# a-to-the-5/Simple-MapReduce-Search-Engine-Information-Retrieval-

Hardware: AMD Instinct MI355X
Metric: index build GB/s of text (top-10 queries/sec in 'query') (higher is better)
Workload: dtype u8 text / int32 postings / f64 weights

## Files before the change

### simple-mapreduce-search-engine-information-retrieval-_amd/csrc/sme_sort.hip

```cpp
#include <hip/hip_runtime.h>

#include "sme_internal.hpp"

namespace sme {
namespace {

#ifndef SME_RSNT
#define SME_RSNT 512
#endif
constexpr int kRsNT = SME_RSNT;
constexpr int kRsWaves = kRsNT / 64;
constexpr int kRsIPL = 16;
constexpr int kRsTile = kRsNT * kRsIPL;
constexpr int kRsWaveItems = 64 * kRsIPL;
constexpr int kRsMaxBits = 11;
constexpr int kRsMaxBins = 1 << kRsMaxBits;
constexpr int kRsBPT = kRsMaxBins / kRsNT;
constexpr int kRsGroups = 1024;
constexpr int kRsScanSums = 1024;
constexpr int kRsOffTiles = 16;

struct RsGroups {
  int64_t tpg;
  int G;
};
static RsGroups rs_groups(int64_t ntiles) {
  const int64_t tpg = std::max<int64_t>(4, (ntiles + kRsGroups - 1) / kRsGroups);
  const int64_t g = (ntiles + tpg - 1) / tpg;
  return RsGroups{tpg, (int)((g + 15) / 16 * 16)};
}

struct Gather {
  const int64_t *reg, *xoff, *crec;
  int64_t nrec;
  const uint32_t *rval;
  int tf_shift;
};
__device__ __forceinline__ void gather_start(const Gather &g, int64_t x, int64_t &rec, int64_t &nx, int64_t &dl) {
  rec = g.crec[x >> 10];
  nx = g.xoff[rec + 1];
  dl = g.reg[rec] - g.xoff[rec];
}
__device__ __forceinline__ int64_t gather_pos(const Gather &g, int64_t x, int64_t &rec, int64_t &nx, int64_t &dl) {
  while (x >= nx) {
    rec++;
    nx = g.xoff[rec + 1];
    dl = g.reg[rec] - g.xoff[rec];
  }
  return x + dl;
}
constexpr int kGRec = 48;
__device__ __forceinline__ int64_t gather_table(const Gather &g, int64_t x0, int lane, int64_t *gx, int64_t *gdl,
                                                uint32_t *gv = nullptr) {
  const int64_t rec0 = g.crec[x0 >> 10];
  const int64_t r = rec0 + lane;
  if (lane < kGRec) {
    gx[lane] = r <= g.nrec ? g.xoff[r] : INT64_MAX;
    gdl[lane] = r < g.nrec ? g.reg[r] - g.xoff[r] : 0;
    if (gv) gv[lane] = r < g.nrec ? g.rval[r] : 0u;
  }
  if (lane == 0) gx[kGRec] = rec0 + kGRec <= g.nrec ? g.xoff[rec0 + kGRec] : INT64_MAX;
  __builtin_amdgcn_fence(__ATOMIC_SEQ_CST, "wavefront");
  __builtin_amdgcn_wave_barrier();
  return rec0;
}
__device__ __forceinline__ int64_t gather_at(const Gather &g, int64_t x, int &j, const int64_t *gx, const int64_t *gdl,
                                             int64_t rec0, uint32_t *jr = nullptr) {
#ifdef SME_RS_GATHER_CEIL
  if (jr) *jr = 0u;
  return x + gdl[0];
#endif
  while (j < kGRec - 1 && x >= gx[j + 1]) j++;
  if (x < gx[j + 1]) {
    if (jr) *jr = (uint32_t)j;
    return x + gdl[j];
  }
  int64_t rec = rec0 + kGRec - 1, nx = g.xoff[rec + 1], dl = g.reg[rec] - g.xoff[rec];
  const int64_t p = gather_pos(g, x, rec, nx, dl);
  if (jr) *jr = (uint32_t)(rec - rec0);
  return p;
}
__global__ void k_rs_chunk_rec(const int64_t *__restrict__ xoff, int64_t nrec, int64_t P, int64_t *__restrict__ crec) {
  for (int64_t c = blockIdx.x * (int64_t)blockDim.x + threadIdx.x; (c << 10) < P; c += (int64_t)gridDim.x * blockDim.x) {
    const int64_t x = c << 10;
    int64_t lo = 0, hi = nrec;
    while (hi - lo > 1) {
      const int64_t m = (lo + hi) >> 1;
      if (xoff[m] <= x) lo = m;
      else hi = m;
    }
    crec[c] = lo;
  }
}

__global__ __launch_bounds__(kRsNT) void k_rs_count(const uint32_t *__restrict__ key, int64_t P, int shift,
                                                    int nbins, uint32_t *__restrict__ counts, Gather g) {
  __shared__ uint32_t h[kRsMaxBins];
  const int tid = threadIdx.x;
  for (int b = tid; b < nbins; b += kRsNT) h[b] = 0;
  __syncthreads();
  const int64_t t0 = (int64_t)blockIdx.x * kRsTile;
  const uint32_t mask = (uint32_t)nbins - 1u;
  const int64_t n = min((int64_t)kRsTile, P - t0);
  if (g.reg != nullptr) {
    __shared__ int64_t gx_all[kRsWaves][kGRec + 1], gdl_all[kRsWaves][kGRec];
    const int lane = tid & 63, w = tid >> 6;
    const int64_t wb = t0 + (int64_t)w * kRsWaveItems;
    if (wb < P) {
      const int64_t rec0 = gather_table(g, wb, lane, gx_all[w], gdl_all[w]);
      int j = 0;
      uint32_t kk[kRsIPL];
#pragma unroll
      for (int s = 0; s < kRsIPL; s++) {
        const int64_t x = wb + s * 64 + lane;
        kk[s] = x < P ? key[gather_at(g, x, j, gx_all[w], gdl_all[w], rec0)] : 0u;
      }
#pragma unroll
      for (int s = 0; s < kRsIPL; s++)
        if (wb + s * 64 + lane < P) atomicAdd(&h[(kk[s] >> shift) & mask], 1u);
    }
  } else if (n == kRsTile) {
    const uint4 *k4 = reinterpret_cast<const uint4 *>(key + t0);
#pragma unroll
    for (int i = 0; i < kRsIPL / 4; i++) {
      const uint4 v = k4[i * kRsNT + tid];
      atomicAdd(&h[(v.x >> shift) & mask], 1u);
      atomicAdd(&h[(v.y >> shift) & mask], 1u);
      atomicAdd(&h[(v.z >> shift) & mask], 1u);
      atomicAdd(&h[(v.w >> shift) & mask], 1u);
    }
  } else {
    for (int64_t i = tid; i < n; i += kRsNT) atomicAdd(&h[(key[t0 + i] >> shift) & mask], 1u);
  }
  __syncthreads();
  for (int b = tid; b < nbins; b += kRsNT) counts[(int64_t)blockIdx.x * nbins + b] = h[b];
}

__global__ __launch_bounds__(kRsNT) void k_rs_colsum(const uint32_t *__restrict__ counts, int64_t ntiles, int nbins,
                                                     int64_t tpg, int G, uint32_t *__restrict__ gsum) {
  const int g = blockIdx.x;
  const int64_t ta = (int64_t)g * tpg, tb = min(ntiles, ta + tpg);
  for (int b = threadIdx.x; b < nbins; b += kRsNT) {
    uint32_t s = 0;
    for (int64_t t = ta; t < tb; t++) s += counts[t * nbins + b];
    gsum[(int64_t)b * G + g] = s;
  }
}

__global__ __launch_bounds__(kRsNT) void k_rs_scan(uint32_t *__restrict__ a, int n) {
  __shared__ uint32_t ws[kRsWaves];
  const int tid = threadIdx.x, lane = tid & 63, w = tid >> 6;
  uint32_t carry = 0;
  uint4 x[4];
  auto load = [&](int r0, uint4 *y) {
    const int i0 = r0 + 16 * tid;
#pragma unroll
    for (int c = 0; c < 4; c++) y[c] = i0 < n ? reinterpret_cast<const uint4 *>(a + i0)[c] : make_uint4(0, 0, 0, 0);
  };
  load(0, x);
  for (int r0 = 0; r0 < n; r0 += 16 * kRsNT) {
    const int i0 = r0 + 16 * tid;
    uint32_t s = 0;
#pragma unroll
    for (int c = 0; c < 4; c++) s += x[c].x + x[c].y + x[c].z + x[c].w;
    uint32_t incl = s;
    for (int o = 1; o < 64; o <<= 1) {
      const uint32_t u = __shfl_up(incl, o, 64);
      if (lane >= o) incl += u;
    }
    if (lane == 63) ws[w] = incl;
    uint4 xn[4];
    load(r0 + 16 * kRsNT, xn);
    __syncthreads();
    uint32_t wb = carry, tot = 0;
    for (int j = 0; j < kRsWaves; j++) {
      const uint32_t t = ws[j];
      if (j < w) wb += t;
      tot += t;
    }
    uint32_t run = wb + incl - s;
    if (i0 < n) {
#pragma unroll
      for (int c = 0; c < 4; c++) {
        uint4 y;
        y.x = run;
        run += x[c].x;
        y.y = run;
        run += x[c].y;
        y.z = run;
        run += x[c].z;
        y.w = run;
        run += x[c].w;
        reinterpret_cast<uint4 *>(a + i0)[c] = y;
      }
    }
    carry += tot;
    __syncthreads();
#pragma unroll
    for (int c = 0; c < 4; c++) x[c] = xn[c];
  }
}

__global__ __launch_bounds__(kRsNT) void k_rs_colscan(uint32_t *__restrict__ counts, int64_t ntiles, int nbins,
                                                      int64_t tpg, int G, const uint32_t *__restrict__ gsum) {
  const int g = blockIdx.x;
  const int64_t ta = (int64_t)g * tpg, tb = min(ntiles, ta + tpg);
  for (int b = threadIdx.x; b < nbins; b += kRsNT) {
    uint32_t run = gsum[(int64_t)b * G + g];
    for (int64_t t = ta; t < tb; t++) {
      const uint32_t c = counts[t * nbins + b];
      counts[t * nbins + b] = run;
      run += c;
    }
  }
}

template <bool LAST, bool PACK, bool KEYS = true>
__global__ __launch_bounds__(kRsNT) void k_rs_scatter(const uint32_t *__restrict__ key, const uint32_t *__restrict__ val,
                                                      int64_t P, int shift, int nbits,
                                                      const uint32_t *__restrict__ offs, uint32_t *__restrict__ okey,
                                                      uint32_t *__restrict__ oval, int32_t *__restrict__ odocno,
                                                      int32_t *__restrict__ otf, int64_t dmin, uint32_t F,
                                                      Gather g, const double *__restrict__ lut, double idf,
                                                      double *__restrict__ ow, const uint2 *__restrict__ xw) {
  __shared__ uint16_t wc[kRsWaves * kRsMaxBins];
  __shared__ uint32_t gd[kRsMaxBins];
  __shared__ uint32_t stage[kRsTile];
  __shared__ uint32_t ws[kRsWaves];
  const int tid = threadIdx.x, lane = tid & 63, w = tid >> 6;
  const int nbins = 1 << nbits;
  const uint32_t mask = (uint32_t)nbins - 1u;
  const int64_t per = (int64_t)(gridDim.x >> 3);
  const int64_t tile = (int64_t)(blockIdx.x & 7) * per + (blockIdx.x >> 3);
  const int64_t t0 = tile * kRsTile;
  if (t0 >= P) return;
  const int n = (int)min((int64_t)kRsTile, P - t0);
  for (int i = tid; i < kRsWaves * kRsMaxBins / 2; i += kRsNT) reinterpret_cast<uint32_t *>(wc)[i] = 0u;
  __syncthreads();
  uint16_t *mine = wc + w * kRsMaxBins;
  const int wb = w * kRsWaveItems;
  const uint64_t lt = (1ull << lane) - 1ull;
  uint32_t k[kRsIPL], v[kRsIPL], pos[kRsIPL];
  if (g.reg != nullptr) {
    __shared__ int64_t gx_all[kRsWaves][kGRec + 1], gdl_all[kRsWaves][kGRec];
    __shared__ uint32_t gv_all[kRsWaves][kGRec];
    uint32_t *gv = PACK ? gv_all[w] : nullptr;
    int64_t rec0 = 0;
    if (wb < n) rec0 = gather_table(g, t0 + wb, lane, gx_all[w], gdl_all[w], gv);
    int j = 0;
    if (PACK) {
      const uint32_t kmask = g.tf_shift >= 32 ? 0xFFFFFFFFu : (1u << g.tf_shift) - 1u;
#pragma unroll
      for (int s = 0; s < kRsIPL; s++) {
        const int i = wb + s * 64 + lane;
        k[s] = 0u;
        v[s] = 0u;
        if (i < n) k[s] = key[gather_at(g, t0 + i, j, gx_all[w], gdl_all[w], rec0, &v[s])];
      }
#pragma unroll
      for (int s = 0; s < kRsIPL; s++) {
        const uint32_t wd = k[s], jr = v[s];
        k[s] = wd & kmask;
        if (wb + s * 64 + lane < n)
          v[s] = (jr < (uint32_t)kGRec ? gv[jr] : g.rval[rec0 + jr]) + (uint32_t)((uint64_t)wd >> g.tf_shift);
      }
    } else {
#pragma unroll
      for (int s = 0; s < kRsIPL; s++) {
        const int i = wb + s * 64 + lane;
        k[s] = 0u;
        v[s] = 0u;
        if (i < n) {
          const int64_t p = gather_at(g, t0 + i, j, gx_all[w], gdl_all[w], rec0);
          k[s] = key[p];
          v[s] = val[p];
        }
      }
    }
  } else {
#pragma unroll
    for (int s = 0; s < kRsIPL; s++) {
      const int i = wb + s * 64 + lane;
      const bool ok = i < n;
      k[s] = ok ? key[t0 + i] : 0u;
      v[s] = ok ? val[t0 + i] : 0u;
    }
  }
#pragma unroll
  for (int s = 0; s < kRsIPL; s++) {
    const bool ok = wb + s * 64 + lane < n;
    const uint32_t d = (k[s] >> shift) & mask;
    uint64_t peers = (uint64_t)__ballot(ok);
    for (int b = 0; b < nbits; b++) {
      const bool bit = (d >> b) & 1u;
      const uint64_t m = (uint64_t)__ballot(bit);
      peers &= bit ? m : ~m;
    }
    uint32_t r = 0;
    if (ok) {
      const uint32_t c = mine[d];
      r = c + (uint32_t)__popcll(peers & lt);
      if ((peers & lt) == 0) mine[d] = (uint16_t)(c + (uint32_t)__popcll(peers));
    }
    pos[s] = r;
  }
  __syncthreads();
  {
    const int b0 = kRsBPT * tid;
    uint32_t tc[kRsBPT];
    uint32_t s2 = 0;
#pragma unroll
    for (int q = 0; q < kRsBPT; q++) {
      tc[q] = 0;
      if (b0 + q < nbins) {
#pragma unroll
        for (int x = 0; x < kRsWaves; x++) tc[q] += wc[x * kRsMaxBins + b0 + q];
      }
      s2 += tc[q];
    }
    uint32_t incl = s2;
    for (int o = 1; o < 64; o <<= 1) {
      const uint32_t u = __shfl_up(incl, o, 64);
      if (lane >= o) incl += u;
    }
    if (lane == 63) ws[w] = incl;
    __syncthreads();
    uint32_t ex = incl - s2;
    for (int j = 0; j < w; j++) ex += ws[j];
#pragma unroll
    for (int q = 0; q < kRsBPT; q++) {
      if (b0 + q < nbins) {
        uint32_t r = ex;
        gd[b0 + q] = offs[tile * nbins + b0 + q] - r;
#pragma unroll
        for (int x = 0; x < kRsWaves; x++) {
          const uint32_t c = wc[x * kRsMaxBins + b0 + q];
          wc[x * kRsMaxBins + b0 + q] = (uint16_t)r;
          r += c;
        }
      }
      ex += tc[q];
    }
  }
  __syncthreads();
#pragma unroll
  for (int s = 0; s < kRsIPL; s++) {
    if (wb + s * 64 + lane >= n) continue;
    pos[s] += mine[(k[s] >> shift) & mask];
    stage[pos[s]] = k[s];
  }
  __syncthreads();
  uint32_t dst[kRsIPL];
#pragma unroll
  for (int j = 0; j < kRsIPL; j++) {
    const int p = j * kRsNT + tid;
    if (p < n) {
      const uint32_t kk = stage[p];
      dst[j] = gd[(kk >> shift) & mask] + (uint32_t)p;
      if (LAST && xw) {
        const uint2 x = xw[kk];
        dst[j] += x.x;
        if (KEYS) okey[dst[j]] = x.y;
      } else if (KEYS) {
        okey[dst[j]] = kk;
      }
    }
  }
  __syncthreads();
#pragma unroll
  for (int s = 0; s < kRsIPL; s++)
    if (wb + s * 64 + lane < n) stage[pos[s]] = v[s];
  __syncthreads();
#pragma unroll
  for (int j = 0; j < kRsIPL; j++) {
    const int p = j * kRsNT + tid;
    if (p < n) {
      const uint32_t vv = stage[p];
      if (LAST) {
        odocno[dst[j]] = (int32_t)((int64_t)(vv / F) + dmin);
        otf[dst[j]] = (int32_t)(vv % F);
        if (ow) ow[dst[j]] = __dmul_rn(lut[vv % F], idf);
      } else {
        oval[dst[j]] = vv;
      }
    }
  }
}

__global__ __launch_bounds__(kRsNT) void k_rs_term_off(const uint32_t *__restrict__ key, int64_t P, int shift, int nbits,
                                                       const uint32_t *__restrict__ offs, int64_t V,
                                                       const uint2 *__restrict__ xw, int64_t *__restrict__ off,
                                                       int64_t vend, int64_t pend) {
  __shared__ uint32_t ks[kRsTile];
  __shared__ uint16_t sp[kRsTile];
  __shared__ uint32_t hist[kRsMaxBins];
  __shared__ uint32_t rc[kRsIPL * kRsWaves + 1];
  __shared__ uint32_t act;
  const int tid = threadIdx.x, lane = tid & 63, w = tid >> 6;
  const int nbins = 1 << nbits;
  const uint32_t mask = (uint32_t)nbins - 1u;
  const uint32_t lmask = (1u << shift) - 1u;
  if (blockIdx.x == 0 && tid == 0) off[vend] = pend;
  if (P <= 0) return;
  int64_t tile = 0;
  auto emit = [&](uint32_t L) {
    for (int d = tid; d < nbins; d += kRsNT) {
      const uint64_t k = ((uint64_t)d << shift) | L;
      if (k < (uint64_t)V) {
        const int64_t o = (int64_t)offs[tile * nbins + d] + hist[d];
        if (xw) {
          const uint2 x = xw[k];
          off[x.y] = o + x.x;
        } else {
          off[k] = o;
        }
      }
    }
  };
  if (shift == 0) {
    for (int b = tid; b < nbins; b += kRsNT) hist[b] = 0;
    __syncthreads();
    emit(0u);
    return;
  }
  if (tid == 0) act = 0u;
  __syncthreads();
  if (tid < kRsOffTiles) {
    const int64_t a0 = ((int64_t)blockIdx.x * kRsOffTiles + tid) * kRsTile;
    if (a0 < P) {
      const int64_t last = min(a0 + kRsTile, P) - 1;
      if (a0 == 0 || (key[a0 - 1] & lmask) != (key[last] & lmask)) atomicOr(&act, 1u << tid);
    }
  }
  __syncthreads();
  const uint64_t lt = (1ull << lane) - 1ull;
  for (uint32_t todo = act; todo != 0u; todo &= todo - 1u) {
    tile = (int64_t)blockIdx.x * kRsOffTiles + (__ffs(todo) - 1);
    const int64_t t0 = tile * kRsTile;
    const int n = (int)min((int64_t)kRsTile, P - t0);
    const uint32_t lprev = t0 > 0 ? key[t0 - 1] & lmask : 0u;
    for (int b = tid; b < nbins; b += kRsNT) hist[b] = 0;
    for (int p = tid; p < n; p += kRsNT) ks[p] = key[t0 + p];
    __syncthreads();
    uint32_t mine = 0;
#pragma unroll
    for (int j = 0; j < kRsIPL; j++) {
      const int p = j * kRsNT + tid;
      bool f = false;
      if (p < n) f = (ks[p] & lmask) != (p > 0 ? ks[p - 1] & lmask : lprev) || (p == 0 && t0 == 0);
      const uint64_t b = (uint64_t)__ballot(f);
      if (f) mine |= 1u << j;
      if (lane == 0) rc[j * kRsWaves + w] = (uint32_t)__popcll(b);
    }
    __syncthreads();
    if (w == 0) {
      const uint32_t a = rc[2 * lane], b = rc[2 * lane + 1];
      uint32_t incl = a + b;
      for (int o = 1; o < 64; o <<= 1) {
        const uint32_t u = __shfl_up(incl, o, 64);
        if (lane >= o) incl += u;
      }
      rc[2 * lane] = incl - a - b;
      rc[2 * lane + 1] = incl - b;
      if (lane == 63) rc[kRsIPL * kRsWaves] = incl;
    }
    __syncthreads();
#pragma unroll
    for (int j = 0; j < kRsIPL; j++) {
      const bool f = (mine >> j) & 1u;
      const uint64_t b = (uint64_t)__ballot(f);
      if (f) sp[rc[j * kRsWaves + w] + (uint32_t)__popcll(b & lt)] = (uint16_t)(j * kRsNT + tid);
    }
    __syncthreads();
    const int ns = (int)rc[kRsIPL * kRsWaves];
    int pos = 0;
    for (int si = 0; si < ns; si++) {
      const int s = sp[si];
      for (int p = pos + tid; p < s; p += kRsNT) atomicAdd(&hist[(ks[p] >> shift) & mask], 1u);
      __syncthreads();
      emit(ks[s] & lmask);
      __syncthreads();
      pos = s;
    }
    __syncthreads();
  }
}

template <typename K>
__global__ __launch_bounds__(kRsNT) void k_kv_count(const K *__restrict__ key, int64_t n, int shift, int nbins,
                                                    uint32_t *__restrict__ counts) {
  __shared__ uint32_t h[kRsMaxBins];
  const int tid = threadIdx.x;
  for (int b = tid; b < nbins; b += kRsNT) h[b] = 0;
  __syncthreads();
  const int64_t t0 = (int64_t)blockIdx.x * kRsTile;
  const int m = (int)min((int64_t)kRsTile, n - t0);
  const uint32_t mask = (uint32_t)nbins - 1u;
  for (int i = tid; i < m; i += kRsNT) atomicAdd(&h[(uint32_t)(key[t0 + i] >> shift) & mask], 1u);
  __syncthreads();
  for (int b = tid; b < nbins; b += kRsNT) counts[(int64_t)blockIdx.x * nbins + b] = h[b];
}

template <typename K, bool KEYS>
__global__ __launch_bounds__(kRsNT) void k_kv_scatter(const K *__restrict__ key, const uint32_t *__restrict__ val,
                                                      int64_t n_all, int shift, int nbits,
                                                      const uint32_t *__restrict__ offs, K *__restrict__ okey,
                                                      uint32_t *__restrict__ oval) {
  __shared__ uint16_t wc[kRsWaves * kRsMaxBins];
  __shared__ uint32_t gd[kRsMaxBins];
  __shared__ uint32_t stage[kRsTile];
  __shared__ uint32_t ws[kRsWaves];
  const int tid = threadIdx.x, lane = tid & 63, w = tid >> 6;
  const int nbins = 1 << nbits;
  const uint32_t mask = (uint32_t)nbins - 1u;
  const int64_t per = (int64_t)(gridDim.x >> 3);
  const int64_t tile = (int64_t)(blockIdx.x & 7) * per + (blockIdx.x >> 3);
  const int64_t t0 = tile * kRsTile;
  if (t0 >= n_all) return;
  const int n = (int)min((int64_t)kRsTile, n_all - t0);
  for (int i = tid; i < kRsWaves * kRsMaxBins / 2; i += kRsNT) reinterpret_cast<uint32_t *>(wc)[i] = 0u;
  __syncthreads();
  uint16_t *mine = wc + w * kRsMaxBins;
  const int wb = w * kRsWaveItems;
  const uint64_t lt = (1ull << lane) - 1ull;
  K k[kRsIPL];
  uint32_t v[kRsIPL], pos[kRsIPL];
#pragma unroll
  for (int s = 0; s < kRsIPL; s++) {
    const int i = wb + s * 64 + lane;
    const bool ok = i < n;
    k[s] = ok ? key[t0 + i] : (K)0;
    v[s] = ok ? val[t0 + i] : 0u;
  }
#pragma unroll
  for (int s = 0; s < kRsIPL; s++) {
    const bool ok = wb + s * 64 + lane < n;
    const uint32_t d = (uint32_t)(k[s] >> shift) & mask;
    uint64_t peers = (uint64_t)__ballot(ok);
    for (int b = 0; b < nbits; b++) {
      const bool bit = (d >> b) & 1u;
      const uint64_t m = (uint64_t)__ballot(bit);
      peers &= bit ? m : ~m;
    }
    uint32_t r = 0;
    if (ok) {
      const uint32_t c = mine[d];
      r = c + (uint32_t)__popcll(peers & lt);
      if ((peers & lt) == 0) mine[d] = (uint16_t)(c + (uint32_t)__popcll(peers));
    }
    pos[s] = r;
  }
  __syncthreads();
  {
    const int b0 = kRsBPT * tid;
    uint32_t tc[kRsBPT];
    uint32_t s2 = 0;
#pragma unroll
    for (int q = 0; q < kRsBPT; q++) {
      tc[q] = 0;
      if (b0 + q < nbins) {
#pragma unroll
        for (int x = 0; x < kRsWaves; x++) tc[q] += wc[x * kRsMaxBins + b0 + q];
      }
      s2 += tc[q];
    }
    uint32_t incl = s2;
    for (int o = 1; o < 64; o <<= 1) {
      const uint32_t u = __shfl_up(incl, o, 64);
      if (lane >= o) incl += u;
    }
    if (lane == 63) ws[w] = incl;
    __syncthreads();
    uint32_t ex = incl - s2;
    for (int j = 0; j < w; j++) ex += ws[j];
#pragma unroll
    for (int q = 0; q < kRsBPT; q++) {
      if (b0 + q < nbins) {
        uint32_t r = ex;
        gd[b0 + q] = offs[tile * nbins + b0 + q] - r;
#pragma unroll
        for (int x = 0; x < kRsWaves; x++) {
          const uint32_t c = wc[x * kRsMaxBins + b0 + q];
          wc[x * kRsMaxBins + b0 + q] = (uint16_t)r;
          r += c;
        }
      }
      ex += tc[q];
    }
  }
  __syncthreads();
#pragma unroll
  for (int s = 0; s < kRsIPL; s++) {
    if (wb + s * 64 + lane >= n) continue;
    pos[s] += mine[(uint32_t)(k[s] >> shift) & mask];
    stage[pos[s]] = (uint32_t)(k[s] >> shift) & mask;
  }
  __syncthreads();
  uint32_t dst[kRsIPL];
#pragma unroll
  for (int j = 0; j < kRsIPL; j++) {
    const int p = j * kRsNT + tid;
    if (p < n) dst[j] = gd[stage[p]] + (uint32_t)p;
  }
  constexpr int kHalves = KEYS ? (int)(sizeof(K) / 4) : 0;
#pragma unroll
  for (int hf = 0; hf <= kHalves; hf++) {
    __syncthreads();
#pragma unroll
    for (int s = 0; s < kRsIPL; s++)
      if (wb + s * 64 + lane < n) stage[pos[s]] = hf < kHalves ? (uint32_t)((uint64_t)k[s] >> (32 * hf)) : v[s];
    __syncthreads();
#pragma unroll
    for (int j = 0; j < kRsIPL; j++) {
      const int p = j * kRsNT + tid;
      if (p < n) {
        if (hf < kHalves) reinterpret_cast<uint32_t *>(okey + dst[j])[hf] = stage[p];
        else oval[dst[j]] = stage[p];
      }
    }
  }
}

constexpr int kScNT = 256, kScIPT = 16, kScTile = kScNT * kScIPT;

template <typename T>
__device__ __forceinline__ T sc_block_excl(T v, T *ws, T *total) {
  const int lane = threadIdx.x & 63, w = threadIdx.x >> 6;
  T incl = v;
  for (int o = 1; o < 64; o <<= 1) {
    const T u = __shfl_up(incl, o, 64);
    if (lane >= o) incl += u;
  }
  if (lane == 63) ws[w] = incl;
  __syncthreads();
  T base = 0, tot = 0;
  for (int j = 0; j < kScNT / 64; j++) {
    if (j < w) base += ws[j];
    tot += ws[j];
  }
  __syncthreads();
  *total = tot;
  return base + incl - v;
}

template <typename T>
__global__ __launch_bounds__(kScNT) void k_sc_sums(const T *__restrict__ in, int64_t n, T *__restrict__ sums) {
  __shared__ T ws[kScNT / 64];
  const int64_t t0 = (int64_t)blockIdx.x * kScTile;
  T s = 0;
#pragma unroll
  for (int j = 0; j < kScIPT; j++) {
    const int64_t i = t0 + j * kScNT + threadIdx.x;
    if (i < n) s += in[i];
  }
  T tot;
  (void)sc_block_excl<T>(s, ws, &tot);
  if (threadIdx.x == 0) sums[blockIdx.x] = tot;
}

template <typename T>
__global__ __launch_bounds__(kScNT) void k_sc_carry(T *__restrict__ a, int64_t n) {
  __shared__ T ws[kScNT / 64];
  T carry = 0;
  for (int64_t r0 = 0; r0 < n; r0 += kScTile) {
    const int64_t i0 = r0 + (int64_t)threadIdx.x * kScIPT;
    T x[kScIPT], s = 0;
#pragma unroll
    for (int j = 0; j < kScIPT; j++) {
      x[j] = i0 + j < n ? a[i0 + j] : (T)0;
      s += x[j];
    }
    T tot;
    T run = carry + sc_block_excl<T>(s, ws, &tot);
#pragma unroll
    for (int j = 0; j < kScIPT; j++) {
      if (i0 + j < n) a[i0 + j] = run;
      run += x[j];
    }
    carry += tot;
  }
}

template <typename T>
__global__ __launch_bounds__(kScNT) void k_sc_apply(const T *in, T *out, int64_t n, const T *__restrict__ carry) {
  __shared__ T st[kScTile + kScTile / 16];
  __shared__ T ws[kScNT / 64];
  auto P = [](int i) { return i + (i >> 4); };
  const int64_t t0 = (int64_t)blockIdx.x * kScTile;
#pragma unroll
  for (int j = 0; j < kScIPT; j++) {
    const int64_t i = t0 + j * kScNT + threadIdx.x;
    st[P(j * kScNT + threadIdx.x)] = i < n ? in[i] : (T)0;
  }
  __syncthreads();
  T x[kScIPT], s = 0;
#pragma unroll
  for (int j = 0; j < kScIPT; j++) {
    x[j] = st[P(threadIdx.x * kScIPT + j)];
    s += x[j];
  }
  T tot;
  T run = carry[blockIdx.x] + sc_block_excl<T>(s, ws, &tot);
#pragma unroll
  for (int j = 0; j < kScIPT; j++) {
    st[P(threadIdx.x * kScIPT + j)] = run;
    run += x[j];
  }
  __syncthreads();
#pragma unroll
  for (int j = 0; j < kScIPT; j++) {
    const int64_t i = t0 + j * kScNT + threadIdx.x;
    if (i < n) out[i] = st[P(j * kScNT + threadIdx.x)];
  }
}

__global__ void k_flags_i64(const uint8_t *__restrict__ f, int64_t n, int64_t *__restrict__ v) {
  for (int64_t i = blockIdx.x * (int64_t)blockDim.x + threadIdx.x; i < n; i += (int64_t)gridDim.x * blockDim.x)
    v[i] = f[i] ? 1 : 0;
}
__global__ void k_select_scatter(const uint8_t *__restrict__ f, const int64_t *__restrict__ pos, int64_t n,
                                 int32_t *__restrict__ out, int32_t *__restrict__ count) {
  for (int64_t i = blockIdx.x * (int64_t)blockDim.x + threadIdx.x; i < n; i += (int64_t)gridDim.x * blockDim.x) {
    if (f[i]) out[pos[i]] = (int32_t)i;
    if (i == n - 1) *count = (int32_t)(pos[i] + (f[i] ? 1 : 0));
  }
}

void rs_scan(uint32_t *gsum, int64_t n, uint32_t *sums, hipStream_t st) {
  if (n <= 16 * 4 * kRsNT) {
    hipLaunchKernelGGL(k_rs_scan, dim3(1), dim3(kRsNT), 0, st, gsum, (int)n);
    return;
  }
  const int64_t nt = (n + kScTile - 1) / kScTile;
  hipLaunchKernelGGL(k_sc_sums<uint32_t>, dim3((unsigned)nt), dim3(kScNT), 0, st, gsum, n, sums);
  hipLaunchKernelGGL(k_sc_carry<uint32_t>, dim3(1), dim3(kScNT), 0, st, sums, nt);
  hipLaunchKernelGGL(k_sc_apply<uint32_t>, dim3((unsigned)nt), dim3(kScNT), 0, st, gsum, gsum, n, sums);
}

}

uint32_t *term_sort(uint32_t *k0, uint32_t *v0, uint32_t *k1, uint32_t *v1, int64_t nrec, const int64_t *reg,
                    const int64_t *xoff, int64_t P, int bits, int64_t dmin, uint32_t F, int32_t *docno, int32_t *tf,
                    uint32_t *counts, hipStream_t st, const double *lut, double idf, double *w, int maxbits,
                    const uint2 *xw, int64_t Pout, const uint32_t *rec_val, int tf_shift, int64_t *off_out, int64_t V,
                    int64_t vend, bool write_keys) {
  if (vend <= 0) vend = V;
  const int64_t pend = xw ? Pout : std::max<int64_t>(P, 0);
  if (P <= 0) {
    if (off_out) {
      hipLaunchKernelGGL(k_rs_term_off, dim3(1), dim3(kRsNT), 0, st, nullptr, 0, 0, 1, nullptr, V, xw, off_out, vend,
                         pend);
      SME_CHECK_LAUNCH();
    }
    return k0;
  }
  if (P > 0xFFFFFFFFll) throw Error(SME_ELIMIT, "term sort of more than 2^32 pairs");
  bits = std::max(bits, 1);
  maxbits = std::min(std::max(maxbits, 1), kRsMaxBits);
  const int npass = term_sort_passes(bits, maxbits);
  const int64_t ntiles = (P + kRsTile - 1) / kRsTile;
  const RsGroups rg = rs_groups(ntiles);
  const int64_t tpg = rg.tpg;
  const int G = rg.G;
  uint32_t *gsum = counts + ntiles * kRsMaxBins;
  Gather g0{nullptr, nullptr, nullptr, 0, nullptr, 0};
  if (reg != nullptr) {
    int64_t *crec = reinterpret_cast<int64_t *>(gsum + kRsMaxBins * kRsGroups + kRsScanSums);
    const int64_t nch = (P + 1023) >> 10;
    hipLaunchKernelGGL(k_rs_chunk_rec, dim3((unsigned)std::min<int64_t>((nch + 255) / 256, 4096)), dim3(256), 0, st,
                       xoff, nrec, P, crec);
    g0 = Gather{reg, xoff, crec, nrec, rec_val, tf_shift};
  }
  int shift = 0;
  for (int p = 0; p < npass; p++) {
    const Gather g = p == 0 ? g0 : Gather{nullptr, nullptr, nullptr, 0, nullptr, 0};
#ifdef SME_RS_LOFIRST
    const int nb = (bits - shift) / (npass - p);
#else
    const int nb = (bits - shift + (npass - p) - 1) / (npass - p);
#endif
    const int nbins = 1 << nb;
    const bool last = p == npass - 1;
    hipLaunchKernelGGL(k_rs_count, dim3((unsigned)ntiles), dim3(kRsNT), 0, st, k0, P, shift, nbins, counts, g);
    hipLaunchKernelGGL(k_rs_colsum, dim3(G), dim3(kRsNT), 0, st, counts, ntiles, nbins, tpg, G, gsum);
    rs_scan(gsum, (int64_t)nbins * G, gsum + kRsMaxBins * kRsGroups, st);
    hipLaunchKernelGGL(k_rs_colscan, dim3(G), dim3(kRsNT), 0, st, counts, ntiles, nbins, tpg, G, gsum);
    const unsigned sgrid = (unsigned)(8 * ((ntiles + 7) / 8));
    if (last && xw && write_keys)
      SME_HIP(hipMemsetAsync(k1, 0xFF, (size_t)Pout * sizeof(uint32_t), st));
    const bool pack = g.reg != nullptr && g.rval != nullptr;
    auto *scatter = !last        ? (pack ? k_rs_scatter<false, true> : k_rs_scatter<false, false>)
                    : write_keys ? (pack ? k_rs_scatter<true, true> : k_rs_scatter<true, false>)
                                 : (pack ? k_rs_scatter<true, true, false> : k_rs_scatter<true, false, false>);
    if (last)
      hipLaunchKernelGGL(scatter, dim3(sgrid), dim3(kRsNT), 0, st, k0, v0, P, shift, nb, counts, k1, nullptr, docno, tf,
                         dmin, F, g, lut, idf, w, xw);
    else
      hipLaunchKernelGGL(scatter, dim3(sgrid), dim3(kRsNT), 0, st, k0, v0, P, shift, nb, counts, k1, v1, nullptr,
                         nullptr, dmin, F, g, nullptr, 0.0, nullptr, nullptr);
    if (last && off_out)
      hipLaunchKernelGGL(k_rs_term_off, dim3(shift == 0 ? 1u : (unsigned)((ntiles + kRsOffTiles - 1) / kRsOffTiles)),
                         dim3(kRsNT), 0, st, k0, P, shift, nb, counts, V, xw, off_out, vend, pend);
    SME_CHECK_LAUNCH();
    std::swap(k0, k1);
    std::swap(v0, v1);
    shift += nb;
  }
  return k0;
}

int term_sort_passes(int bits, int maxbits) {
  const int mb = std::min(std::max(maxbits, 1), kRsMaxBits);
  return (std::max(bits, 1) + mb - 1) / mb;
}

size_t term_sort_scratch(int64_t P) {
  const int64_t ntiles = (std::max<int64_t>(P, 1) + kRsTile - 1) / kRsTile;
  return (size_t)(ntiles * kRsMaxBins + (int64_t)kRsMaxBins * kRsGroups + kRsScanSums) * sizeof(uint32_t) +
         (size_t)(((std::max<int64_t>(P, 1) + 1023) >> 10) + 1) * sizeof(int64_t);
}
template <typename K>
uint32_t *kv_sort(K *k0, uint32_t *v0, K *k1, uint32_t *v1, int64_t n, int bits, uint32_t *scratch, hipStream_t st,
                  bool keys_out) {
  if (n <= 1) return v0;
  if (n > 0xFFFFFFFFll) throw Error(SME_ELIMIT, "sort of more than 2^32 pairs");
  bits = std::min(std::max(bits, 1), (int)(8 * sizeof(K)));
  const int npass = (bits + kRsMaxBits - 1) / kRsMaxBits;
  const int64_t ntiles = (n + kRsTile - 1) / kRsTile;
  const RsGroups rg = rs_groups(ntiles);
  const int64_t tpg = rg.tpg;
  const int G = rg.G;
  uint32_t *counts = scratch, *gsum = scratch + ntiles * kRsMaxBins;
  int shift = 0;
  for (int p = 0; p < npass; p++) {
    const int nb = (bits - shift + (npass - p) - 1) / (npass - p);
    const int nbins = 1 << nb;
    hipLaunchKernelGGL(k_kv_count<K>, dim3((unsigned)ntiles), dim3(kRsNT), 0, st, k0, n, shift, nbins, counts);
    hipLaunchKernelGGL(k_rs_colsum, dim3(G), dim3(kRsNT), 0, st, counts, ntiles, nbins, tpg, G, gsum);
    rs_scan(gsum, (int64_t)nbins * G, gsum + kRsMaxBins * kRsGroups, st);
    hipLaunchKernelGGL(k_rs_colscan, dim3(G), dim3(kRsNT), 0, st, counts, ntiles, nbins, tpg, G, gsum);
    const unsigned sgrid = (unsigned)(8 * ((ntiles + 7) / 8));
    if (p == npass - 1 && !keys_out)
      hipLaunchKernelGGL((k_kv_scatter<K, false>), dim3(sgrid), dim3(kRsNT), 0, st, k0, v0, n, shift, nb, counts,
                         k1, v1);
    else
      hipLaunchKernelGGL((k_kv_scatter<K, true>), dim3(sgrid), dim3(kRsNT), 0, st, k0, v0, n, shift, nb, counts, k1,
                         v1);
    SME_CHECK_LAUNCH();
    std::swap(k0, k1);
    std::swap(v0, v1);
    shift += nb;
  }
  return v0;
}
template uint32_t *kv_sort<uint64_t>(uint64_t *, uint32_t *, uint64_t *, uint32_t *, int64_t, int, uint32_t *,
                                     hipStream_t, bool);
template uint32_t *kv_sort<uint32_t>(uint32_t *, uint32_t *, uint32_t *, uint32_t *, int64_t, int, uint32_t *,
                                     hipStream_t, bool);

namespace {
__global__ void k_sp_iota(uint32_t *a, int64_t n) {
  for (int64_t i = blockIdx.x * (int64_t)blockDim.x + threadIdx.x; i < n; i += (int64_t)gridDim.x * blockDim.x)
    a[i] = (uint32_t)i;
}
__global__ void k_sp_gather64(const uint64_t *__restrict__ v, const uint32_t *__restrict__ idx, int64_t n,
                              uint64_t *__restrict__ out) {
  for (int64_t i = blockIdx.x * (int64_t)blockDim.x + threadIdx.x; i < n; i += (int64_t)gridDim.x * blockDim.x)
    out[i] = v[idx[i]];
}
template <typename T>
__global__ void k_max_zero(T *m) {
  *m = 0;
}
__device__ __forceinline__ void atomic_max_t(int32_t *p, int32_t v) { atomicMax(p, v); }
__device__ __forceinline__ void atomic_max_t(int64_t *p, int64_t v) {
  atomicMax(reinterpret_cast<unsigned long long *>(p), (unsigned long long)v);
}
template <typename T>
__global__ void k_max_reduce(const T *__restrict__ in, int64_t n, T *m) {
  T x = 0;
  for (int64_t i = blockIdx.x * (int64_t)blockDim.x + threadIdx.x; i < n; i += (int64_t)gridDim.x * blockDim.x)
    x = in[i] > x ? in[i] : x;
  for (int o = 32; o > 0; o >>= 1) {
    const T y = __shfl_xor(x, o, 64);
    x = y > x ? y : x;
  }
  if ((threadIdx.x & 63) == 0 && x > 0) atomic_max_t(m, x);
}
__global__ void k_run_heads(const uint64_t *__restrict__ k, int64_t n, int64_t *__restrict__ f) {
  for (int64_t i = blockIdx.x * (int64_t)blockDim.x + threadIdx.x; i <= n; i += (int64_t)gridDim.x * blockDim.x)
    f[i] = (i < n && (i == 0 || k[i] != k[i - 1])) ? 1 : 0;
}
__global__ void k_run_sums(const uint64_t *__restrict__ k, const int32_t *__restrict__ v, int64_t n,
                           const int64_t *__restrict__ f, const int64_t *__restrict__ pos, uint64_t *__restrict__ uk,
                           int32_t *__restrict__ sums, int64_t *d_runs) {
  for (int64_t i = blockIdx.x * (int64_t)blockDim.x + threadIdx.x; i < n; i += (int64_t)gridDim.x * blockDim.x) {
    const int64_t r = pos[i] + f[i] - 1;
    if (f[i]) uk[r] = k[i];
    atomicAdd(&sums[r], v[i]);
    if (i == n - 1) *d_runs = r + 1;
  }
}
unsigned sp_grid(int64_t n) { return (unsigned)std::max<int64_t>(1, std::min<int64_t>((n + 255) / 256, 16384)); }
}

template <typename K>
void sort_pairs(K *keys_in, K *keys_out, uint32_t *vals_in, uint32_t *vals_out, int64_t n, int bits, DevBuf &radix,
                hipStream_t st) {
  if (n <= 0) return;
  uint32_t *scr = radix.as<uint32_t>(kv_sort_scratch(n) / sizeof(uint32_t) + 1);
  if (kv_sort<K>(keys_in, vals_in, keys_out, vals_out, n, bits, scr, st, true) == vals_in) {
    SME_HIP(hipMemcpyAsync(keys_out, keys_in, (size_t)n * sizeof(K), hipMemcpyDeviceToDevice, st));
    SME_HIP(hipMemcpyAsync(vals_out, vals_in, (size_t)n * sizeof(uint32_t), hipMemcpyDeviceToDevice, st));
  }
}
template void sort_pairs<uint64_t>(uint64_t *, uint64_t *, uint32_t *, uint32_t *, int64_t, int, DevBuf &,
                                   hipStream_t);
template void sort_pairs<uint32_t>(uint32_t *, uint32_t *, uint32_t *, uint32_t *, int64_t, int, DevBuf &,
                                   hipStream_t);
template <typename K>
void sort_pairs_v64(K *keys_in, K *keys_out, const uint64_t *vals_in, uint64_t *vals_out, int64_t n, int bits,
                    DevBuf &ia, DevBuf &ib, DevBuf &radix, hipStream_t st) {
  if (n <= 0) return;
  uint32_t *a = ia.as<uint32_t>((size_t)n + 1), *b = ib.as<uint32_t>((size_t)n + 1);
  hipLaunchKernelGGL(k_sp_iota, dim3(sp_grid(n)), dim3(256), 0, st, a, n);
  sort_pairs<K>(keys_in, keys_out, a, b, n, bits, radix, st);
  if (vals_in) hipLaunchKernelGGL(k_sp_gather64, dim3(sp_grid(n)), dim3(256), 0, st, vals_in, b, n, vals_out);
  SME_CHECK_LAUNCH();
}
template void sort_pairs_v64<uint64_t>(uint64_t *, uint64_t *, const uint64_t *, uint64_t *, int64_t, int, DevBuf &,
                                       DevBuf &, DevBuf &, hipStream_t);
template void sort_pairs_v64<uint32_t>(uint32_t *, uint32_t *, const uint64_t *, uint64_t *, int64_t, int, DevBuf &,
                                       DevBuf &, DevBuf &, hipStream_t);
template <typename T>
void reduce_max(const T *in, int64_t n, T *d_max, hipStream_t st) {
  hipLaunchKernelGGL(k_max_zero<T>, dim3(1), dim3(1), 0, st, d_max);
  if (n > 0) hipLaunchKernelGGL(k_max_reduce<T>, dim3(std::min(sp_grid(n), 2048u)), dim3(256), 0, st, in, n, d_max);
  SME_CHECK_LAUNCH();
}
template void reduce_max<int32_t>(const int32_t *, int64_t, int32_t *, hipStream_t);
template void reduce_max<int64_t>(const int64_t *, int64_t, int64_t *, hipStream_t);
void reduce_by_key_sum(const uint64_t *keys, const int32_t *vals, int64_t n, uint64_t *ukeys, int32_t *sums,
                       int64_t *d_runs, DevBuf &flags, DevBuf &pos, DevBuf &scan, hipStream_t st) {
  if (n <= 0) {
    SME_HIP(hipMemsetAsync(d_runs, 0, sizeof(int64_t), st));
    return;
  }
  int64_t *f = flags.as<int64_t>((size_t)n + 1), *p = pos.as<int64_t>((size_t)n + 1);
  hipLaunchKernelGGL(k_run_heads, dim3(sp_grid(n + 1)), dim3(256), 0, st, keys, n, f);
  excl_scan(f, p, n + 1, scan, st);
  SME_HIP(hipMemsetAsync(sums, 0, (size_t)n * sizeof(int32_t), st));
  hipLaunchKernelGGL(k_run_sums, dim3(sp_grid(n)), dim3(256), 0, st, keys, vals, n, f, p, ukeys, sums, d_runs);
  SME_CHECK_LAUNCH();
}

template <typename T>
void excl_scan(const T *in, T *out, int64_t n, DevBuf &scratch, hipStream_t st) {
  if (n <= 0) return;
  const int64_t nt = (n + kScTile - 1) / kScTile;
  T *sums = scratch.as<T>((size_t)nt + 1);
  hipLaunchKernelGGL(k_sc_sums<T>, dim3((unsigned)nt), dim3(kScNT), 0, st, in, n, sums);
  hipLaunchKernelGGL(k_sc_carry<T>, dim3(1), dim3(kScNT), 0, st, sums, nt);
  hipLaunchKernelGGL(k_sc_apply<T>, dim3((unsigned)nt), dim3(kScNT), 0, st, in, out, n, (const T *)sums);
  SME_CHECK_LAUNCH();
}
template void excl_scan<int64_t>(const int64_t *, int64_t *, int64_t, DevBuf &, hipStream_t);
template void excl_scan<int32_t>(const int32_t *, int32_t *, int64_t, DevBuf &, hipStream_t);
template void excl_scan<uint32_t>(const uint32_t *, uint32_t *, int64_t, DevBuf &, hipStream_t);

void select_flagged(const uint8_t *flag, int64_t n, int32_t *out, int32_t *d_count, DevBuf &s1, DevBuf &s2,
                    hipStream_t st) {
  if (n <= 0) {
    SME_HIP(hipMemsetAsync(d_count, 0, sizeof(int32_t), st));
    return;
  }
  int64_t *pos = s1.as<int64_t>((size_t)n);
  const unsigned g = (unsigned)std::min<int64_t>((n + 255) / 256, 16384);
  hipLaunchKernelGGL(k_flags_i64, dim3(g), dim3(256), 0, st, flag, n, pos);
  excl_scan<int64_t>(pos, pos, n, s2, st);
  hipLaunchKernelGGL(k_select_scatter, dim3(g), dim3(256), 0, st, flag, pos, n, out, d_count);
  SME_CHECK_LAUNCH();
}

size_t kv_sort_scratch(int64_t n) {
  const int64_t ntiles = (std::max<int64_t>(n, 1) + kRsTile - 1) / kRsTile;
  return (size_t)(ntiles * kRsMaxBins + (int64_t)kRsMaxBins * kRsGroups + kRsScanSums) * sizeof(uint32_t);
}
}
```

Before: 182.6.

## Replace per-lane linear record search with wave-wide bitmap-and-popcount gather tables

```diff
diff --git a/simple-mapreduce-search-engine-information-retrieval-_amd/csrc/sme_sort.hip b/simple-mapreduce-search-engine-information-retrieval-_amd/csrc/sme_sort.hip
--- a/simple-mapreduce-search-engine-information-retrieval-_amd/csrc/sme_sort.hip
+++ b/simple-mapreduce-search-engine-information-retrieval-_amd/csrc/sme_sort.hip
@@ -36,11 +36,6 @@
   const uint32_t *rval;
   int tf_shift;
 };
-__device__ __forceinline__ void gather_start(const Gather &g, int64_t x, int64_t &rec, int64_t &nx, int64_t &dl) {
-  rec = g.crec[x >> 10];
-  nx = g.xoff[rec + 1];
-  dl = g.reg[rec] - g.xoff[rec];
-}
 __device__ __forceinline__ int64_t gather_pos(const Gather &g, int64_t x, int64_t &rec, int64_t &nx, int64_t &dl) {
   while (x >= nx) {
     rec++;
@@ -49,36 +44,82 @@
   }
   return x + dl;
 }
-constexpr int kGRec = 48;
-__device__ __forceinline__ int64_t gather_table(const Gather &g, int64_t x0, int lane, int64_t *gx, int64_t *gdl,
-                                                uint32_t *gv = nullptr) {
-  const int64_t rec0 = g.crec[x0 >> 10];
-  const int64_t r = rec0 + lane;
-  if (lane < kGRec) {
-    gx[lane] = r <= g.nrec ? g.xoff[r] : INT64_MAX;
-    gdl[lane] = r < g.nrec ? g.reg[r] - g.xoff[r] : 0;
-    if (gv) gv[lane] = r < g.nrec ? g.rval[r] : 0u;
-  }
-  if (lane == 0) gx[kGRec] = rec0 + kGRec <= g.nrec ? g.xoff[rec0 + kGRec] : INT64_MAX;
+constexpr int kGScan = 256;
+struct __attribute__((may_alias)) GatherTab {
+  unsigned long long m[kRsIPL];
+  int64_t dl[kGScan];
+  uint32_t bv[kGScan];
+};
+__device__ __forceinline__ int64_t wave_lane_i64(int64_t v, int src) {
+  const uint32_t lo = (uint32_t)__builtin_amdgcn_readlane((int)(uint32_t)v, src);
+  const uint32_t hi = (uint32_t)__builtin_amdgcn_readlane((int)(uint32_t)((uint64_t)v >> 32), src);
+  return (int64_t)(((uint64_t)hi << 32) | lo);
+}
+struct GatherWave {
+  int64_t rend, xlim;
+};
+__device__ __forceinline__ GatherWave gather_fill(const Gather &g, int64_t x0, int lane, GatherTab *t, bool bq) {
+  const int64_t rec0 = g.crec[x0 >> 10], xend = x0 + kRsWaveItems;
+  const uint64_t lt = (1ull << lane) - 1ull;
+  if (lane < kRsIPL) t->m[lane] = 0ull;
   __builtin_amdgcn_fence(__ATOMIC_SEQ_CST, "wavefront");
   __builtin_amdgcn_wave_barrier();
-  return rec0;
-}
-__device__ __forceinline__ int64_t gather_at(const Gather &g, int64_t x, int &j, const int64_t *gx, const int64_t *gdl,
-                                             int64_t rec0, uint32_t *jr = nullptr) {
-#ifdef SME_RS_GATHER_CEIL
-  if (jr) *jr = 0u;
-  return x + gdl[0];
-#endif
-  while (j < kGRec - 1 && x >= gx[j + 1]) j++;
-  if (x < gx[j + 1]) {
-    if (jr) *jr = (uint32_t)j;
-    return x + gdl[j];
-  }
-  int64_t rec = rec0 + kGRec - 1, nx = g.xoff[rec + 1], dl = g.reg[rec] - g.xoff[rec];
-  const int64_t p = gather_pos(g, x, rec, nx, dl);
-  if (jr) *jr = (uint32_t)(rec - rec0);
-  return p;
+  int64_t rend = rec0, xlim;
+  int nq = 1;
+  do {
+    const int64_t r = rend + lane, rc = min(r, g.nrec - 1);
+    const bool in = r < g.nrec;
+    const int64_t xs = g.xoff[rc], xn = g.xoff[rc + 1], rg = g.reg[rc];
+    const uint32_t b = bq ? g.rval[rc] : 0u;
+    const int64_t xe = in ? xn : INT64_MAX;
+    const bool own = in && xn > xs && xs > x0 && xs < xend;
+    const uint64_t ob = (uint64_t)__ballot(own);
+    if (own || r == rec0) {
+      const int q = own ? nq + (int)__popcll(ob & lt) : 0;
+      t->dl[q] = rg - xs;
+      if (bq) t->bv[q] = b;
+      if (own) atomicOr(&t->m[(xs - x0) >> 6], 1ull << ((xs - x0) & 63));
+    }
+    nq += (int)__popcll(ob);
+    rend += 64;
+    xlim = wave_lane_i64(xe, 63);
+  } while (xlim < xend && rend - rec0 < kGScan);
+  __builtin_amdgcn_fence(__ATOMIC_SEQ_CST, "wavefront");
+  __builtin_amdgcn_wave_barrier();
+  return GatherWave{rend, xlim};
+}
+template <int S0, int NS>
+__device__ __forceinline__ uint32_t gather_addr(const Gather &g, int64_t x0, int64_t P, int lane, const GatherTab *t,
+                                                const GatherWave &gw, int64_t (&a)[NS], uint32_t *bq) {
+  const int64_t mv = (int64_t)t->m[lane & (kRsIPL - 1)];
+  const uint64_t le = ((1ull << lane) - 1ull) | (1ull << lane);
+  int pre = 0;
+#pragma unroll
+  for (int s = 0; s < S0 + NS; s++) {
+    const uint64_t mw = (uint64_t)wave_lane_i64(mv, s);
+    if (s >= S0) {
+      const int q = pre + (int)__popcll(mw & le);
+      a[s - S0] = x0 + s * 64 + lane + t->dl[q];
+      if (bq) bq[s - S0] = (uint32_t)q;
+    }
+    pre += (int)__popcll(mw);
+  }
+  uint32_t walked = 0u;
+  if (gw.xlim < min(x0 + kRsWaveItems, P)) {
+#pragma unroll
+    for (int s = S0; s < S0 + NS; s++) {
+      const int64_t x = x0 + s * 64 + lane;
+      if (x >= gw.xlim && x < P) {
+        int64_t rec = gw.rend - 1, nx = gw.xlim, dl = 0;
+        a[s - S0] = gather_pos(g, x, rec, nx, dl);
+        if (bq) {
+          bq[s - S0] = g.rval[rec];
+          walked |= 1u << s;
+        }
+      }
+    }
+  }
+  return walked;
 }
 __global__ void k_rs_chunk_rec(const int64_t *__restrict__ xoff, int64_t nrec, int64_t P, int64_t *__restrict__ crec) {
   for (int64_t c = blockIdx.x * (int64_t)blockDim.x + threadIdx.x; (c << 10) < P; c += (int64_t)gridDim.x * blockDim.x) {
@@ -103,18 +144,20 @@
   const uint32_t mask = (uint32_t)nbins - 1u;
   const int64_t n = min((int64_t)kRsTile, P - t0);
   if (g.reg != nullptr) {
-    __shared__ int64_t gx_all[kRsWaves][kGRec + 1], gdl_all[kRsWaves][kGRec];
+    __shared__ GatherTab gt_all[kRsWaves];
     const int lane = tid & 63, w = tid >> 6;
     const int64_t wb = t0 + (int64_t)w * kRsWaveItems;
     if (wb < P) {
-      const int64_t rec0 = gather_table(g, wb, lane, gx_all[w], gdl_all[w]);
-      int j = 0;
+      const GatherWave gw = gather_fill(g, wb, lane, &gt_all[w], false);
       uint32_t kk[kRsIPL];
-#pragma unroll
-      for (int s = 0; s < kRsIPL; s++) {
-        const int64_t x = wb + s * 64 + lane;
-        kk[s] = x < P ? key[gather_at(g, x, j, gx_all[w], gdl_all[w], rec0)] : 0u;
-      }
+      constexpr int kH = kRsIPL / 2;
+      int64_t a[kH];
+      gather_addr<0, kH>(g, wb, P, lane, &gt_all[w], gw, a, nullptr);
+#pragma unroll
+      for (int s = 0; s < kH; s++) kk[s] = wb + s * 64 + lane < P ? key[a[s]] : 0u;
+      gather_addr<kH, kH>(g, wb, P, lane, &gt_all[w], gw, a, nullptr);
+#pragma unroll
+      for (int s = kH; s < kRsIPL; s++) kk[s] = wb + s * 64 + lane < P ? key[a[s - kH]] : 0u;
 #pragma unroll
       for (int s = 0; s < kRsIPL; s++)
         if (wb + s * 64 + lane < P) atomicAdd(&h[(kk[s] >> shift) & mask], 1u);
@@ -225,7 +268,7 @@
                                                       double *__restrict__ ow, const uint2 *__restrict__ xw) {
   __shared__ uint16_t wc[kRsWaves * kRsMaxBins];
   __shared__ uint32_t gd[kRsMaxBins];
-  __shared__ uint32_t stage[kRsTile];
+  __shared__ __align__(16) uint32_t stage[kRsTile];
   __shared__ uint32_t ws[kRsWaves];
   const int tid = threadIdx.x, lane = tid & 63, w = tid >> 6;
   const int nbins = 1 << nbits;
@@ -242,38 +285,36 @@
   const uint64_t lt = (1ull << lane) - 1ull;
   uint32_t k[kRsIPL], v[kRsIPL], pos[kRsIPL];
   if (g.reg != nullptr) {
-    __shared__ int64_t gx_all[kRsWaves][kGRec + 1], gdl_all[kRsWaves][kGRec];
-    __shared__ uint32_t gv_all[kRsWaves][kGRec];
-    uint32_t *gv = PACK ? gv_all[w] : nullptr;
-    int64_t rec0 = 0;
-    if (wb < n) rec0 = gather_table(g, t0 + wb, lane, gx_all[w], gdl_all[w], gv);
-    int j = 0;
+    static_assert(kRsWaves * sizeof(GatherTab) <= sizeof(stage), "the gather tables alias stage");
+    GatherTab *gt = reinterpret_cast<GatherTab *>(stage) + w;
+    int64_t a[kRsIPL];
+#pragma unroll
+    for (int s = 0; s < kRsIPL; s++) {
+      a[s] = 0;
+      k[s] = 0u;
+      v[s] = 0u;
+    }
     if (PACK) {
       const uint32_t kmask = g.tf_shift >= 32 ? 0xFFFFFFFFu : (1u << g.tf_shift) - 1u;
+      uint32_t walked = 0u;
+      if (wb < n) walked = gather_addr<0, kRsIPL>(g, t0 + wb, P, lane, gt, gather_fill(g, t0 + wb, lane, gt, true), a, v);
+#pragma unroll
+      for (int s = 0; s < kRsIPL; s++)
+        if (wb + s * 64 + lane < n) k[s] = key[a[s]];
 #pragma unroll
       for (int s = 0; s < kRsIPL; s++) {
-        const int i = wb + s * 64 + lane;
-        k[s] = 0u;
-        v[s] = 0u;
-        if (i < n) k[s] = key[gather_at(g, t0 + i, j, gx_all[w], gdl_all[w], rec0, &v[s])];
-      }
-#pragma unroll
-      for (int s = 0; s < kRsIPL; s++) {
-        const uint32_t wd = k[s], jr = v[s];
+        const uint32_t wd = k[s], q = v[s];
         k[s] = wd & kmask;
         if (wb + s * 64 + lane < n)
-          v[s] = (jr < (uint32_t)kGRec ? gv[jr] : g.rval[rec0 + jr]) + (uint32_t)((uint64_t)wd >> g.tf_shift);
+          v[s] = ((walked >> s) & 1u ? q : gt->bv[q]) + (uint32_t)((uint64_t)wd >> g.tf_shift);
       }
     } else {
+      if (wb < n) gather_addr<0, kRsIPL>(g, t0 + wb, P, lane, gt, gather_fill(g, t0 + wb, lane, gt, false), a, nullptr);
 #pragma unroll
       for (int s = 0; s < kRsIPL; s++) {
-        const int i = wb + s * 64 + lane;
-        k[s] = 0u;
-        v[s] = 0u;
-        if (i < n) {
-          const int64_t p = gather_at(g, t0 + i, j, gx_all[w], gdl_all[w], rec0);
-          k[s] = key[p];
-          v[s] = val[p];
+        if (wb + s * 64 + lane < n) {
+          k[s] = key[a[s]];
+          v[s] = val[a[s]];
         }
       }
     }
```

Measured after the change: 185.5 (median of 6 runs). +1.6%, better.
